# StarRocks/starrocks

Measured on NVIDIA B200. Metric: rows/sec for SSB Q4.1 hash-join+agg, higher is better.
Workload: dtype int32 keys / int64 sums

## Files before the change

### include/sr_gpu_ops.h

```cpp
#ifndef SR_GPU_OPS_H
#define SR_GPU_OPS_H

#include <stddef.h>
#include <stdint.h>

#ifdef __cplusplus
extern "C" {
#endif

#define SR_ABI_VERSION 1

typedef enum sr_status {
    SR_OK = 0,
    SR_ERR_INVALID_ARGUMENT = -1,
    SR_ERR_NOT_SUPPORTED = -2,
    SR_ERR_OUT_OF_MEMORY = -3,
    SR_ERR_CUDA = -4,
    SR_ERR_STATE = -5,
    SR_ERR_NO_DEVICE = -6
} sr_status;

typedef enum sr_type {
    SR_TYPE_BOOLEAN = 1,
    SR_TYPE_TINYINT = 2,
// ... 299 lines not shown
typedef struct sr_frag_join {
    sr_join* join;
    int32_t probe_key_slot;
    int32_t num_payload;
    int32_t payload_build_slots[SR_MAX_FRAG_PAYLOAD];
} sr_frag_join;

typedef struct sr_fragment_desc {
    sr_scan_desc scan;
    int32_t num_joins;
    int32_t mode_hint;
    sr_frag_join joins[SR_MAX_FRAG_JOINS];
    sr_agg_desc agg;
} sr_fragment_desc;

typedef struct sr_fragment sr_fragment;

sr_fragment* sr_fragment_create(sr_ctx* ctx, const sr_fragment_desc* desc);
void sr_fragment_destroy(sr_fragment* frag);
int32_t sr_fragment_push(sr_fragment* frag, const sr_chunk_view* fact);
sr_agg* sr_fragment_agg(sr_fragment* frag);
typedef struct sr_fragment_plan {
    int32_t num_joins;
    int32_t order[SR_MAX_FRAG_JOINS];
    int32_t bitmap_in_smem[SR_MAX_FRAG_JOINS];
    double pass_rate[SR_MAX_FRAG_JOINS];
    int32_t smem_bytes;
    int32_t grid;
    int32_t block;
    int32_t agg_in_smem;
    int32_t mode;
    int32_t num_stream_joins;
    int32_t num_gather_passes;
    int32_t reserved;
    double pred_rate;
} sr_fragment_plan;
int32_t sr_fragment_get_plan(sr_fragment* frag, sr_fragment_plan* plan);
int32_t sr_fragment_last_pass_ms(sr_fragment* frag, float ms[3]);
int32_t sr_fragment_reset(sr_fragment* frag);
int64_t sr_fragment_rows_passed(sr_fragment* frag);

typedef enum sr_hash_fn { SR_HASH_FNV = 0, SR_HASH_CRC32 = 1, SR_HASH_XXH3 = 2 } sr_hash_fn;
typedef enum sr_reduce_op { SR_REDUCE_MULHI = 0 , SR_REDUCE_MODULO = 1  } sr_reduce_op;

#define SR_MAX_PART_KEYS 4

typedef struct sr_part_desc {
    int32_t hash_fn;
    int32_t reduce_op;
    int32_t num_channels;
    int32_t num_part_slots;
    int32_t part_slots[SR_MAX_PART_KEYS];
} sr_part_desc;

typedef struct sr_xchg sr_xchg;

sr_xchg* sr_xchg_create(sr_ctx* ctx, const sr_part_desc* desc);
void sr_xchg_destroy(sr_xchg* x);
int32_t sr_xchg_partition(sr_xchg* x, const sr_chunk_view* in, sr_chunk_out* out, int64_t* channel_offsets_host);
int32_t sr_xchg_hash(sr_xchg* x, const sr_chunk_view* in, uint32_t* hash_values, uint32_t* channel_ids, int32_t mem);

typedef enum sr_page_encoding {
    SR_PAGE_PLAIN = 0,
    SR_PAGE_FOR = 1
} sr_page_encoding;

typedef struct sr_page_view {
// ... 52 lines not shown
```

### starrocks_b200/abi.py

```python
import ctypes as C

import numpy as np

SR_ABI_VERSION = 1

SR_OK = 0
SR_ERR_INVALID_ARGUMENT = -1
SR_ERR_NOT_SUPPORTED = -2
SR_ERR_OUT_OF_MEMORY = -3
SR_ERR_CUDA = -4
SR_ERR_STATE = -5
SR_ERR_NO_DEVICE = -6

TYPE_BOOLEAN, TYPE_TINYINT, TYPE_SMALLINT, TYPE_INT, TYPE_BIGINT, TYPE_LARGEINT = 1, 2, 3, 4, 5, 6
TYPE_FLOAT, TYPE_DOUBLE, TYPE_DATE, TYPE_DATETIME = 7, 8, 9, 10
TYPE_DECIMAL32, TYPE_DECIMAL64, TYPE_DECIMAL128 = 11, 12, 13

TYPE_WIDTH = {
    TYPE_BOOLEAN: 1, TYPE_TINYINT: 1, TYPE_SMALLINT: 2, TYPE_INT: 4, TYPE_BIGINT: 8, TYPE_LARGEINT: 16,
    TYPE_FLOAT: 4, TYPE_DOUBLE: 8, TYPE_DATE: 4, TYPE_DATETIME: 8, TYPE_DECIMAL32: 4, TYPE_DECIMAL64: 8,
    TYPE_DECIMAL128: 16,
}
TYPE_NUMPY = {
    TYPE_BOOLEAN: np.uint8, TYPE_TINYINT: np.int8, TYPE_SMALLINT: np.int16, TYPE_INT: np.int32,
# ... 101 lines not shown
    _fields_ = [("method", C.c_int32), ("has_duplicates", C.c_int32), ("build_rows", C.c_int64),
                ("bucket_size", C.c_int64), ("min_value", C.c_int64), ("max_value", C.c_int64)]


class sr_agg_fn(C.Structure):
    _fields_ = [("kind", C.c_int32), ("input_type", C.c_int32), ("out_slot", C.c_int32), ("reserved", C.c_int32),
                ("input", sr_expr)]


class sr_agg_desc(C.Structure):
    _fields_ = [("num_group_keys", C.c_int32), ("group_slots", C.c_int32 * SR_MAX_GROUP_KEYS),
                ("group_types", C.c_int32 * SR_MAX_GROUP_KEYS), ("has_ranges", C.c_int32),
                ("group_nullable", C.c_int32 * SR_MAX_GROUP_KEYS),
                ("group_min", C.c_int64 * SR_MAX_GROUP_KEYS), ("group_max", C.c_int64 * SR_MAX_GROUP_KEYS),
                ("num_fns", C.c_int32), ("reserved", C.c_int32), ("fns", sr_agg_fn * SR_MAX_AGG_FNS),
                ("expected_groups", C.c_int64)]


class sr_frag_join(C.Structure):
    _fields_ = [("join", C.c_void_p), ("probe_key_slot", C.c_int32), ("num_payload", C.c_int32),
                ("payload_build_slots", C.c_int32 * SR_MAX_FRAG_PAYLOAD)]


class sr_fragment_desc(C.Structure):
    _fields_ = [("scan", sr_scan_desc), ("num_joins", C.c_int32), ("mode_hint", C.c_int32),
                ("joins", sr_frag_join * SR_MAX_FRAG_JOINS), ("agg", sr_agg_desc)]


class sr_fragment_plan(C.Structure):
    _fields_ = [("num_joins", C.c_int32), ("order", C.c_int32 * SR_MAX_FRAG_JOINS),
                ("bitmap_in_smem", C.c_int32 * SR_MAX_FRAG_JOINS), ("pass_rate", C.c_double * SR_MAX_FRAG_JOINS),
                ("smem_bytes", C.c_int32), ("grid", C.c_int32), ("block", C.c_int32), ("agg_in_smem", C.c_int32),
                ("mode", C.c_int32), ("num_stream_joins", C.c_int32), ("num_gather_passes", C.c_int32),
                ("reserved", C.c_int32), ("pred_rate", C.c_double)]


class sr_part_desc(C.Structure):
    _fields_ = [("hash_fn", C.c_int32), ("reduce_op", C.c_int32), ("num_channels", C.c_int32),
                ("num_part_slots", C.c_int32), ("part_slots", C.c_int32 * SR_MAX_PART_KEYS)]


class sr_rf_info(C.Structure):
    _fields_ = [("min_value", C.c_int64), ("max_value", C.c_int64), ("num_inserted", C.c_int64), ("has_null", C.c_int32),
                ("log_num_buckets", C.c_int32), ("key_type", C.c_int32), ("num_in_values", C.c_int32)]


class sr_scan_rf_stats(C.Structure):
    _fields_ = [("rows_tested", C.c_int64), ("rows_passed", C.c_int64), ("batches_skipped", C.c_int64), ("last_selectivity", C.c_double)]


RF_IN_FILTER_ROW_LIMIT = 1024


STATE_REDUCE_SUM, STATE_REDUCE_MIN, STATE_REDUCE_MAX = 0, 1, 2


class sr_agg_state_array(C.Structure):
    _fields_ = [("data", C.c_void_p), ("count", C.c_int64), ("elem_type", C.c_int32), ("reduce", C.c_int32)]


class Chunk:

    def __init__(self, columns, num_rows=None, mem=MEM_HOST):
        self._keep = []
        self.slots = []
        self.types = []
        cols = (sr_col_view * max(1, len(columns)))()
# ... 234 lines not shown
```

### starrocks_b200/csrc/sr_frag.cuh

```cuda
#pragma once

#include "sr_agg.cuh"

#include "sr_frag_kernel.cuh"
#include "sr_frag_pass.cuh"

struct sr_fragment {
    sr_ctx* ctx = nullptr;
    std::vector<sr_pred> preds;
    std::vector<sr_expr> exprs;
    int32_t num_joins = 0;
    sr_frag_join joins[SR_MAX_FRAG_JOINS];
    sr_agg* agg = nullptr;
    bool compiled = false;
    VReg reg;
    std::vector<int32_t> value_src;
    std::vector<const BuildCol*> value_col;
    srd::FragDev host;
    DevBuf dev, counters;
    Staged staged;
    size_t smem_bytes = 0;
    int32_t queue_word_off = 0;
    bool smem_agg = false;
    int grid = 0;
    int order[SR_MAX_FRAG_JOINS];
    double pass_rate[SR_MAX_FRAG_JOINS];
    double pred_rate = 1.0;
    int force_mode = 0;
    bool selective = false;
    bool expand = false;
    srd::PassDev pass;
    std::vector<int> gather_joins;
    DevBuf sel[2], pass_counters;
    double est_rate = 1.0;
    size_t stream_smem = 0;
    int stream_grid = 0;
    int final_grid = 0;
    cudaEvent_t ev[4] = {nullptr, nullptr, nullptr, nullptr};
    bool timed_push = false;
    ~sr_fragment() {
        for (int e = 0; e < 4; e++)
            if (ev[e]) cudaEventDestroy(ev[e]);
    }
};

struct FragTypeCtx {
    sr_fragment* f;
};

static int32_t frag_slot_type(void* user, int32_t slot) {
    sr_fragment* f = ((FragTypeCtx*)user)->f;
    const int k = f->staged.find(slot);
    if (k >= 0) return f->staged.cols[k].type;
    for (int j = 0; j < f->num_joins; j++)
        for (int p = 0; p < f->joins[j].num_payload; p++)
            if (f->joins[j].payload_build_slots[p] == slot) {
                const BuildCol* bc = f->joins[j].join->find_col(slot);
                return bc ? bc->type : 0;
            }
    return 0;
}
static bool frag_slot_nullable(void* user, int32_t slot) {
    sr_fragment* f = ((FragTypeCtx*)user)->f;
    const int k = f->staged.find(slot);
    if (k >= 0) return f->staged.cols[k].nulls != nullptr;
    for (int j = 0; j < f->num_joins; j++)
        for (int p = 0; p < f->joins[j].num_payload; p++)
            if (f->joins[j].payload_build_slots[p] == slot) {
                const BuildCol* bc = f->joins[j].join->find_col(slot);
                return bc && bc->nullable;
// ... 67 lines not shown
        for (size_t k = 0; k < f->agg->reg.slots.size(); k++) {
            remap[k] = merged.add(f->agg->reg.slots[k], f->agg->reg.types[k]);
            if (remap[k] >= SR_MAX_VALUES) return sr_fail(ctx, SR_ERR_NOT_SUPPORTED, "too many distinct columns");
        }
        srd::AggDev& ah = f->agg->host;
        for (int k = 0; k < ah.num_keys; k++) ah.key_value_id[k] = remap[ah.key_value_id[k]];
        for (int q = 0; q < ah.num_fns; q++)
            for (int k = 0; k < ah.fns[q].input.num_nodes; k++)
                if (ah.fns[q].input.nodes[k].op == srd::C_LOAD_I || ah.fns[q].input.nodes[k].op == srd::C_LOAD_D)
                    ah.fns[q].input.nodes[k].arg = remap[ah.fns[q].input.nodes[k].arg];
        f->agg->reg = merged;
        f->reg = merged;
        SR_TRY(agg_upload(f->agg));
    }
    f->value_src.assign(f->reg.slots.size(), -1);
    f->value_col.assign(f->reg.slots.size(), nullptr);
    for (size_t k = 0; k < f->reg.slots.size(); k++) {
        if (f->staged.find(f->reg.slots[k]) >= 0) continue;
        bool found = false;
        for (int j = 0; j < f->num_joins && !found; j++)
            for (int p = 0; p < f->joins[j].num_payload && !found; p++)
                if (f->joins[j].payload_build_slots[p] == f->reg.slots[k]) {
                    f->value_src[k] = j;
                    f->value_col[k] = f->joins[j].join->find_col(f->reg.slots[k]);
                    h.joins[j].need_head = 1;
                    found = true;
                }
        if (!found) return sr_fail(ctx, SR_ERR_INVALID_ARGUMENT, "slot %d is neither a fact column nor a join payload", f->reg.slots[k]);
    }
    SR_TRY(f->counters.reserve(ctx, 256));
    SR_CUDA(ctx, cudaMemsetAsync(f->counters.p, 0, 256, ctx->stream));
    h.rows_passed = f->counters.as<unsigned long long>();
    return SR_OK;
}

static int32_t frag_plan(sr_fragment* f, const VTab& vt, int64_t n) {
    sr_ctx* ctx = f->ctx;
    srd::FragDev& h = f->host;
    SR_TRY(f->dev.reserve(ctx, sizeof(srd::FragDev)));
    SR_CUDA(ctx, cudaMemcpyAsync(f->dev.p, &h, sizeof(h), cudaMemcpyHostToDevice, ctx->stream));
    const int64_t sample = std::min<int64_t>(n, 1 << 16);
    unsigned long long counts[24] = {0};
    static_assert(SR_MAX_FRAG_JOINS + 1 <= 16, "sample counter layout");
    counts[SR_MAX_FRAG_JOINS] = (unsigned long long)sample;
    for (int p = 0; p < 8; p++) counts[16 + p] = (unsigned long long)sample;
    if (sample > 0 && (f->num_joins > 0 || h.num_preds > 0 || h.num_exprs > 0)) {
        unsigned long long* dcounts = f->counters.as<unsigned long long>() + 8;
        SR_CUDA(ctx, cudaMemsetAsync(dcounts, 0, sizeof(counts), ctx->stream));
        srd::k_frag_sample<<<grid_for(sample, 256), 256, 0, ctx->stream>>>((const srd::FragDev*)f->dev.p, vt, sample, dcounts);
        SR_LAUNCH_CHECK(ctx);
        SR_CUDA(ctx, cudaMemcpyAsync(counts, dcounts, sizeof(counts), cudaMemcpyDeviceToHost, ctx->stream));
        SR_CUDA(ctx, cudaStreamSynchronize(ctx->stream));
    }
    for (int j = 0; j < f->num_joins; j++) f->pass_rate[j] = sample > 0 ? (double)counts[j] / (double)sample : 1.0;
    f->pred_rate = sample > 0 ? (double)counts[SR_MAX_FRAG_JOINS] / (double)sample : 1.0;
    std::vector<int> ord(f->num_joins);
    for (int j = 0; j < f->num_joins; j++) ord[j] = j;
    std::stable_sort(ord.begin(), ord.end(), [&](int a, int b) {
        const double pa = f->pass_rate[a], pb = f->pass_rate[b];
        if (std::abs(pa - pb) > 0.15 * std::max(pa, pb)) return pa < pb;
        return h.joins[a].bitmap_words < h.joins[b].bitmap_words;
    });
    srd::FragJoinDev reordered[SR_MAX_FRAG_JOINS];
    std::vector<int> inv(f->num_joins);
    for (int q = 0; q < f->num_joins; q++) {
        reordered[q] = h.joins[ord[q]];
// ... 98 lines not shown
            srd::FragJoinDev& fj = h.joins[q];
            fj.smem_off = -1;
            if (q < ns && fj.use_bitmap && sw + (size_t)fj.bitmap_words + 1 <= sbudget) {
                fj.smem_off = (int32_t)sw;
                sw += ((size_t)fj.bitmap_words + 1 + 3) & ~(size_t)3;
            }
        }
        f->stream_smem = sw * 4;
        f->smem_agg = f->agg->smem_bytes > 0;
        f->smem_bytes = f->agg->smem_bytes;
        f->queue_word_off = 0;
        SR_CUDA(ctx, cudaMemcpyAsync(f->dev.p, &h, sizeof(h), cudaMemcpyHostToDevice, ctx->stream));
        SR_CUDA(ctx, cudaStreamSynchronize(ctx->stream));
        int per_sm = 0;
        SR_CUDA(ctx, cudaFuncSetAttribute(srd::k_frag_stream<false>, cudaFuncAttributeMaxDynamicSharedMemorySize, (int)std::max<size_t>(f->stream_smem, 16)));
        SR_CUDA(ctx, cudaFuncSetAttribute(srd::k_frag_stream<true>, cudaFuncAttributeMaxDynamicSharedMemorySize, (int)std::max<size_t>(f->stream_smem, 16)));
        SR_CUDA(ctx, cudaFuncSetAttribute(srd::k_frag_stream_tests<false>, cudaFuncAttributeMaxDynamicSharedMemorySize, (int)std::max<size_t>(f->stream_smem, 16)));
        SR_CUDA(ctx, cudaFuncSetAttribute(srd::k_frag_stream_tests<true>, cudaFuncAttributeMaxDynamicSharedMemorySize, (int)std::max<size_t>(f->stream_smem, 16)));
        SR_CUDA(ctx, cudaOccupancyMaxActiveBlocksPerMultiprocessor(&per_sm, srd::k_frag_stream<false>, srd::STREAM_BLOCK, f->stream_smem));
        if (per_sm < 1) return sr_fail(ctx, SR_ERR_CUDA, "streaming pass does not fit on an SM (smem %zu)", f->stream_smem);
        f->stream_grid = per_sm * ctx->num_sms;
        int gj = 0, ga = 0;
        SR_CUDA(ctx, cudaOccupancyMaxActiveBlocksPerMultiprocessor(&gj, srd::k_frag_gather_join, srd::GATHER_BLOCK, 0));
        if (f->expand)
            SR_CUDA(ctx, cudaOccupancyMaxActiveBlocksPerMultiprocessor(&ga, srd::k_frag_gather_agg_expand, srd::GATHER_BLOCK, 0));
        else if (f->agg->host.num_keys == 0)
            SR_CUDA(ctx, cudaOccupancyMaxActiveBlocksPerMultiprocessor(&ga, srd::k_frag_gather_agg<false, true>, srd::GATHER_BLOCK, 0));
        else if (f->smem_agg)
            SR_CUDA(ctx, cudaOccupancyMaxActiveBlocksPerMultiprocessor(&ga, srd::k_frag_gather_agg<true>, srd::GATHER_BLOCK, f->agg->smem_bytes));
        else
            SR_CUDA(ctx, cudaOccupancyMaxActiveBlocksPerMultiprocessor(&ga, srd::k_frag_gather_agg<false>, srd::GATHER_BLOCK, 0));
        f->grid = std::max(gj, 1) * ctx->num_sms;
        f->final_grid = std::max(ga, 1) * ctx->num_sms;
        SR_TRY(f->pass_counters.reserve(ctx, 16 * sizeof(uint64_t)));
        f->compiled = true;
        return SR_OK;
    }
    size_t words = 0;
    f->smem_agg = f->agg->smem_bytes > 0;
    if (f->smem_agg) words += (f->agg->smem_bytes + 15) / 16 * 4;
    const size_t budget_words = (96 * 1024) / 4;
    const size_t queue_words = (size_t)srd::FRAG_WARPS * srd::FRAG_WARP_QWORDS;
    for (int q = 0; q < f->num_joins; q++) {
        srd::FragJoinDev& fj = h.joins[q];
        fj.smem_off = -1;
        if (fj.use_bitmap && words + (size_t)fj.bitmap_words + queue_words <= budget_words) {
            fj.smem_off = (int32_t)words;
            words += (size_t)fj.bitmap_words;
            words = (words + 3) & ~(size_t)3;
        }
    }
    f->queue_word_off = (int32_t)words;
    words += queue_words;
    f->smem_bytes = words * 4;
    SR_CUDA(ctx, cudaMemcpyAsync(f->dev.p, &h, sizeof(h), cudaMemcpyHostToDevice, ctx->stream));
    SR_CUDA(ctx, cudaStreamSynchronize(ctx->stream));
    int per_sm = 0;
    SR_CUDA(ctx, cudaFuncSetAttribute(srd::k_fragment<true>, cudaFuncAttributeMaxDynamicSharedMemorySize, (int)f->smem_bytes));
    SR_CUDA(ctx, cudaFuncSetAttribute(srd::k_fragment<false>, cudaFuncAttributeMaxDynamicSharedMemorySize, (int)f->smem_bytes));
    if (f->smem_agg)
        SR_CUDA(ctx, cudaOccupancyMaxActiveBlocksPerMultiprocessor(&per_sm, srd::k_fragment<true>, srd::FRAG_BLOCK, f->smem_bytes));
    else
        SR_CUDA(ctx, cudaOccupancyMaxActiveBlocksPerMultiprocessor(&per_sm, srd::k_fragment<false>, srd::FRAG_BLOCK, f->smem_bytes));
    if (per_sm < 1) return sr_fail(ctx, SR_ERR_CUDA, "fragment kernel does not fit on an SM (smem %zu)", f->smem_bytes);
    f->grid = per_sm * ctx->num_sms;
    f->compiled = true;
    return SR_OK;
}

static int32_t frag_push(sr_fragment* f, const sr_chunk_view* fact) {
    sr_ctx* ctx = f->ctx;
    if (f->agg->finished) return sr_fail(ctx, SR_ERR_STATE, "fragment push after sink_finish");
    if (fact->num_rows >= 0xFFFFFFF0ll) return sr_fail(ctx, SR_ERR_NOT_SUPPORTED, "fragment batch of more than 2^32 rows; push smaller morsels");
    SR_TRY(f->staged.stage(ctx, fact, nullptr, true));
    const int64_t n = fact->num_rows;
    bool first = !f->compiled;
    if (first) SR_TRY(frag_compile(f));
    VTab vt;
    SR_TRY(frag_bind_vtab(f, &vt));
    if (first) {
        SR_TRY(frag_plan(f, vt, n));
        SR_TRY(frag_bind_vtab(f, &vt));
    }
    if (n == 0) return SR_OK;
    SR_TRY(agg_check_nullability(f->agg, vt));
// ... 21 lines not shown
        if (!carry) pass.carry_join = pass.carry_value_id = -1;
        unsigned long long* cnt = f->pass_counters.as<unsigned long long>();
        SR_CUDA(ctx, cudaMemsetAsync(cnt, 0, 16 * sizeof(uint64_t), ctx->stream));
        const int sgrid = (int)std::min<int64_t>(f->stream_grid, (n + srd::STREAM_TILE - 1) / srd::STREAM_TILE);
        if (!f->ev[0])
            for (int e = 0; e < 4; e++) SR_CUDA(ctx, cudaEventCreate(&f->ev[e]));
        SR_CUDA(ctx, cudaEventRecord(f->ev[0], ctx->stream));
        bool tests = pass.num_tests > 0;
        for (int t = 0; t < pass.num_tests && tests; t++) {
            const VDesc& d = vt.v[pass.tests[t].value_id];
            if (d.nulls != nullptr || (t < pass.num_vec && (((uintptr_t)d.data) & 15) != 0)) tests = false;
        }
        static const bool use_tma = getenv("SR_FRAG_STREAM_TMA") != nullptr;
        if (tests && use_tma && !pass.host_input) {
            const uint32_t bitmap_bytes = (uint32_t)((f->stream_smem + 127) / 128 * 128);
            const size_t sm = bitmap_bytes + srd::STREAM_TMA_SMEM;
            SR_CUDA(ctx, cudaFuncSetAttribute(srd::k_frag_stream_tests_tma<false>, cudaFuncAttributeMaxDynamicSharedMemorySize, (int)sm));
            int per_sm = 1;
            SR_CUDA(ctx, cudaOccupancyMaxActiveBlocksPerMultiprocessor(&per_sm, srd::k_frag_stream_tests_tma<false>, srd::STREAM_BLOCK, sm));
            const int tgrid = (int)std::min<int64_t>((int64_t)std::max(per_sm, 1) * ctx->num_sms, (n + srd::STREAM_TILE - 1) / srd::STREAM_TILE);
            srd::k_frag_stream_tests_tma<false><<<tgrid, srd::STREAM_BLOCK, sm, ctx->stream>>>(fdev, pass, vt, n, bitmap_bytes, f->sel[0].as<srd::SelEntry>(), cnt);
        } else if (tests) {
            if (carry)
                srd::k_frag_stream_tests<true><<<sgrid, srd::STREAM_BLOCK, f->stream_smem, ctx->stream>>>(fdev, pass, vt, n, f->sel[0].as<srd::SelEntry>(), cnt);
            else
                srd::k_frag_stream_tests<false><<<sgrid, srd::STREAM_BLOCK, f->stream_smem, ctx->stream>>>(fdev, pass, vt, n, f->sel[0].as<srd::SelEntry>(), cnt);
        } else if (carry) {
            srd::k_frag_stream<true><<<sgrid, srd::STREAM_BLOCK, f->stream_smem, ctx->stream>>>(fdev, pass, vt, n, f->sel[0].as<srd::SelEntry>(), cnt);
        } else {
            srd::k_frag_stream<false><<<sgrid, srd::STREAM_BLOCK, f->stream_smem, ctx->stream>>>(fdev, pass, vt, n, f->sel[0].as<srd::SelEntry>(), cnt);
        }
        SR_LAUNCH_CHECK(ctx);
        SR_CUDA(ctx, cudaEventRecord(f->ev[1], ctx->stream));
        int cur = 0, k = 0;
        for (int q : f->gather_joins) {
            srd::k_frag_gather_join<<<f->grid, srd::GATHER_BLOCK, 0, ctx->stream>>>(fdev, q, vt, f->sel[cur].as<srd::SelEntry>(), cnt + k,
                                                                                  f->sel[cur ^ 1].as<srd::SelEntry>(), cnt + k + 1);
            SR_LAUNCH_CHECK(ctx);
            cur ^= 1;
            k++;
        }
        SR_CUDA(ctx, cudaEventRecord(f->ev[2], ctx->stream));
        if (hash) SR_TRY(f->sel[cur ^ 1].reserve(ctx, sizeof(srd::SelEntry) * ((size_t)n + slack)));
        srd::SelEntry* fail_list = hash ? f->sel[cur ^ 1].as<srd::SelEntry>() : nullptr;
        unsigned long long* fail_count = cnt + 8;
        if (f->expand)
            srd::k_frag_gather_agg_expand<<<f->final_grid, srd::GATHER_BLOCK, 0, ctx->stream>>>(fdev, (const srd::AggDev*)a->dev.p, pass, vt,
                                                                                       f->sel[cur].as<srd::SelEntry>(), cnt + k, fail_list, fail_count);
        else if (ah.num_keys == 0)
            srd::k_frag_gather_agg<false, true><<<f->final_grid, srd::GATHER_BLOCK, 0, ctx->stream>>>(fdev, (const srd::AggDev*)a->dev.p, pass, vt,
                                                                                              f->sel[cur].as<srd::SelEntry>(), cnt + k, nullptr, nullptr);
        else if (f->smem_agg)
            srd::k_frag_gather_agg<true><<<f->final_grid, srd::GATHER_BLOCK, a->smem_bytes, ctx->stream>>>(fdev, (const srd::AggDev*)a->dev.p, pass, vt,
                                                                                                   f->sel[cur].as<srd::SelEntry>(), cnt + k, nullptr, nullptr);
        else
            srd::k_frag_gather_agg<false><<<f->final_grid, srd::GATHER_BLOCK, 0, ctx->stream>>>(fdev, (const srd::AggDev*)a->dev.p, pass, vt,
                                                                                        f->sel[cur].as<srd::SelEntry>(), cnt + k, fail_list, fail_count);
        SR_LAUNCH_CHECK(ctx);
        SR_CUDA(ctx, cudaEventRecord(f->ev[3], ctx->stream));
        f->timed_push = true;
        if (hash) {
            int fc = 8;
            while (true) {
                uint64_t ng;
                int32_t ovf, bad;
                SR_CUDA(ctx, cudaMemcpyAsync(ctx->pinned + 16, cnt + fc, 8, cudaMemcpyDeviceToHost, ctx->stream));
                SR_TRY(agg_read_counters(a, &ng, &ovf, &bad));
                a->ngroups_host = (int64_t)ng;
                const uint64_t failed = ctx->pinned[16];
                if (failed == 0) break;
                SR_CUDA(ctx, cudaMemsetAsync((uint8_t*)a->counters.p + 8, 0, 8, ctx->stream));
                uint64_t cap = a->host.cap * 2;
                while ((uint64_t)a->ngroups_host + failed > cap / 2) cap *= 2;
                if (cap > (1ull << 33)) return sr_fail(ctx, SR_ERR_OUT_OF_MEMORY, "aggregate table would exceed 2^33 slots; push smaller batches");
                SR_TRY(agg_grow(a, cap));
                cur ^= 1;
                const int nfc = fc == 8 ? 9 : 8;
                SR_CUDA(ctx, cudaMemsetAsync(cnt + nfc, 0, 8, ctx->stream));
                if (f->expand)
// ... 31 lines not shown
```

### starrocks_b200/csrc/sr_frag_pass.cuh

```cuda
#pragma once

#include "sr_frag_kernel.cuh"

namespace srd {

struct StreamTest {
    int32_t kind;
    int32_t value_id;
    int32_t join;
    uint32_t lo, span;
};
#define SR_MAX_STREAM_TESTS 6

struct PassDev {
    int32_t num_tests;
    int32_t num_vec;
    StreamTest tests[SR_MAX_STREAM_TESTS];
    int32_t num_stream_joins;
    int32_t final_first_join;
    int8_t final_vals[8];
    int8_t final_slot[SR_MAX_VALUES];
    int8_t host_input;
    int8_t carry_join;
    int8_t carry_value_id;
// ... 692 lines not shown
                if (test && head == 0) ok = false;
            } else if (test) {
                if (!join_hit_global(fj, key)) ok = false;
            }
        }
        if (!ok) continue;
        if (single) {
            single_acc_row(ad, sacc, ld);
        } else if (hash_table) {
            HKey key;
            agg_pack_key(ad, ld, key);
            bool inserted;
            const long long slot = agg_find_slot_key(ad, key, inserted, known_groups);
            agg_count_new_groups(ad, inserted, known_groups);
            if (slot < 0) {
                if (fail_list) fail_list[atomicAdd(fail_count, 1ull)] = entry;
                continue;
            }
            agg_apply_row<SMEM_AGG>(ad, acc, slot, ld);
        } else {
            const long long slot = agg_find_slot(ad, ld);
            if (slot >= 0) agg_apply_row<SMEM_AGG>(ad, acc, slot, ld);
        }
        passed++;
    }
    __syncwarp();
    if (single) single_acc_flush(ad, sacc);
    if (SMEM_AGG) {
        __syncthreads();
        acc_smem_flush(ad, acc);
    }
    passed = warp_sum(passed);
    if (lane_id() == 0 && passed) atomicAdd(fd.rows_passed, passed);
}

__global__ void __launch_bounds__(GATHER_BLOCK) k_frag_gather_agg_expand(const FragDev* __restrict__ fdp, const AggDev* __restrict__ adp, const __grid_constant__ PassDev pd,
                                                                          const __grid_constant__ VTab vt, const SelEntry* __restrict__ sel_in,
                                                                          const unsigned long long* __restrict__ n_in_ptr, SelEntry* __restrict__ fail_list,
                                                                          unsigned long long* __restrict__ fail_count) {
    __shared__ FragJoinDev s_joins[SR_MAX_FRAG_JOINS];
    const FragDev& fd = *fdp;
    const AggDev& ad = *adp;
    const int S = fd.num_joins;
    const bool single = ad.num_keys == 0;
    const bool hash_table = !ad.dense && ad.num_keys > 0;
    unsigned long long known_groups = hash_table && fail_list ? *(volatile unsigned long long*)ad.ngroups : 0ull;
    for (int i = threadIdx.x; i < (int)(sizeof(FragJoinDev) / 4) * S; i += blockDim.x) ((uint32_t*)s_joins)[i] = ((const uint32_t*)fd.joins)[i];
    AccPtrs acc;
    acc_ptrs_global(ad, acc);
    __syncthreads();
    const unsigned long long n_in = *n_in_ptr;
    unsigned long long passed = 0;
    SingleAcc sacc;
    if (single) single_acc_init(ad, sacc);
    unsigned long long w_begin, w_end;
    warp_sel_range(n_in, w_begin, w_end);
    for (unsigned long long i = w_begin + lane_id(); i < w_end; i += 32) {
        const SelEntry entry = sel_in[i];
        const uint32_t row = sel_row(entry);
        if (row == SEL_INVALID) continue;
        FragLoader ld{vt, (int64_t)row, {0, 0, 0, 0, 0, 0}, pd.carry_join >= 0 ? (int32_t)pd.carry_value_id : -1, sel_carry(entry)};
        uint32_t head[SR_MAX_FRAG_JOINS];
        bool ok = true;
#pragma unroll 1
        for (int j = 0; j < S && ok; j++) {
            const FragJoinDev& fj = s_joins[j];
// ... 69 lines not shown
```

### starrocks_b200/csrc/sr_gpu.cu

```cuda
#include "sr_frag.cuh"
#include "sr_serde.cuh"
#include "sr_page.cuh"

namespace srd {

struct PartCols {
    DCol c[SR_MAX_PART_KEYS];
    int32_t n;
    int32_t hash_fn;
    int32_t reduce;
    int32_t num_channels;
};

__device__ __forceinline__ uint32_t part_hash_row(const PartCols& pc, int64_t row) {
    uint32_t h = pc.hash_fn == SR_HASH_FNV ? 0x811C9DC5u : pc.hash_fn == SR_HASH_XXH3 ? 0x9E3779B1u : 0u;
    for (int k = 0; k < pc.n; k++) {
        const DCol& c = pc.c[k];
        if (c.nulls && c.nulls[row]) {
            if (pc.hash_fn == SR_HASH_CRC32)
                h = zlib_crc32_bytes(0, 0, 4, h);
            else
                h = h ^ (0x9e3779b9u + (h << 6) + (h >> 2));
            continue;
        }
// ... 1271 lines not shown
    delete frag->agg;
    delete frag;
}

int32_t sr_fragment_push(sr_fragment* frag, const sr_chunk_view* fact) {
    if (!frag || !fact) return SR_ERR_INVALID_ARGUMENT;
    SR_BIND(frag->ctx);
    return frag_push(frag, fact);
}

sr_agg* sr_fragment_agg(sr_fragment* frag) {
    return frag ? frag->agg : nullptr;
}

int32_t sr_fragment_get_plan(sr_fragment* frag, sr_fragment_plan* plan) {
    if (!frag || !plan) return SR_ERR_INVALID_ARGUMENT;
    SR_LOCK(frag->ctx);
    if (!frag->compiled) return sr_fail(frag->ctx, SR_ERR_STATE, "the fragment plans on its first push");
    memset(plan, 0, sizeof(*plan));
    plan->num_joins = frag->num_joins;
    for (int q = 0; q < frag->num_joins; q++) {
        plan->order[q] = frag->order[q];
        plan->bitmap_in_smem[q] = frag->host.joins[q].smem_off >= 0 ? 1 : 0;
        plan->pass_rate[q] = frag->pass_rate[q];
    }
    plan->smem_bytes = (int32_t)frag->smem_bytes;
    plan->grid = frag->grid;
    plan->block = srd::FRAG_BLOCK;
    plan->agg_in_smem = frag->smem_agg ? 1 : 0;
    plan->mode = frag->selective ? 2 : 1;
    plan->num_stream_joins = frag->selective ? frag->pass.num_stream_joins : 0;
    plan->num_gather_passes = frag->selective ? (int32_t)frag->gather_joins.size() : 0;
    plan->pred_rate = frag->pred_rate;
    if (frag->selective) {
        plan->smem_bytes = (int32_t)frag->stream_smem;
        plan->grid = frag->stream_grid;
        plan->block = srd::STREAM_BLOCK;
    }
    return SR_OK;
}

int32_t sr_fragment_last_pass_ms(sr_fragment* frag, float ms[3]) {
    if (!frag || !ms) return SR_ERR_INVALID_ARGUMENT;
    sr_ctx* ctx = frag->ctx;
    SR_BIND(ctx);
    if (!frag->timed_push) return sr_fail(ctx, SR_ERR_STATE, "no timed push (selection-vector mode only)");
    SR_CUDA(ctx, cudaEventSynchronize(frag->ev[3]));
    for (int k = 0; k < 3; k++) SR_CUDA(ctx, cudaEventElapsedTime(&ms[k], frag->ev[k], frag->ev[k + 1]));
    return SR_OK;
}

int32_t sr_fragment_reset(sr_fragment* frag) {
    if (!frag) return SR_ERR_INVALID_ARGUMENT;
    sr_ctx* ctx = frag->ctx;
    SR_BIND(ctx);
    SR_TRY(agg_reset_impl(frag->agg));
    if (frag->compiled) SR_CUDA(ctx, cudaMemsetAsync(frag->counters.p, 0, 8, ctx->stream));
    return SR_OK;
}

int64_t sr_fragment_rows_passed(sr_fragment* frag) {
    if (!frag) return SR_ERR_INVALID_ARGUMENT;
    sr_ctx* ctx = frag->ctx;
    SR_BIND(ctx);
    if (!frag->compiled) return 0;
    SR_CUDA(ctx, cudaMemcpyAsync(ctx->pinned + 16, frag->counters.p, 8, cudaMemcpyDeviceToHost, ctx->stream));
// ... 273 lines not shown
```

### starrocks_b200/gpu.py

```python
import ctypes as C
import os
import subprocess

import numpy as np

from . import abi

_HERE = os.path.dirname(os.path.abspath(__file__))
LIB_PATH = os.environ.get("SR_GPU_LIB") or os.path.join(_HERE, "libsr_gpu.so")
_LIB = None

NVCC_FLAGS = ["-gencode", "arch=compute_100a,code=sm_100a", "-O3", "-lineinfo", "-std=c++17", "-shared",
              "-Xcompiler", "-fPIC", "-cudart", "static"]


def _source_files():
    csrc = os.path.join(_HERE, "csrc")
    return sorted(os.path.join(csrc, f) for f in os.listdir(csrc)) + [os.path.join(_HERE, "..", "include", "sr_gpu_ops.h")]


def _source_hash():
    import hashlib
    h = hashlib.sha256()
    for f in _source_files():
# ... 442 lines not shown
    def num_groups(self):
        return self.ctx.check(lib().sr_agg_num_groups(self.h))

    def pull(self, max_rows=1 << 62, mem=abi.MEM_HOST):
        out = abi.sr_chunk_out()
        self.ctx.check(lib().sr_agg_pull(self.h, max_rows, mem, C.byref(out)))
        return out

    def result(self):
        self.finish()
        out = self.pull()
        return chunk_out_to_host(self.ctx, out)


def two_phase_descs(desc):
    p1, p2 = abi.sr_agg_desc(), abi.sr_agg_desc()
    rc = lib().sr_agg_two_phase_descs(C.byref(desc), C.byref(p1), C.byref(p2))
    if rc != 0:
        raise GpuError(rc, "sr_agg_two_phase_descs: the aggregate cannot be split into two phases (128-bit states or too many functions)")
    return p1, p2


def chunk_out_as_view(out):
    class _View:
        pass
    v = _View()
    v.view = abi.sr_chunk_view(C.cast(out.cols, C.POINTER(abi.sr_col_view)), out.num_cols, out.mem, out.num_rows)
    v.num_rows = out.num_rows
    v._keep = out
    v.ref = lambda: C.byref(v.view)
    return v


class Fragment:
    def __init__(self, ctx, scan_desc, joins, agg_desc, mode=0):
        self.ctx = ctx
        self._keep = (scan_desc, joins, agg_desc)
        d = abi.sr_fragment_desc()
        d.scan = scan_desc.desc
        d.num_joins = len(joins)
        d.mode_hint = mode
        for k, (j, slot, payload) in enumerate(joins):
            d.joins[k].join = j.h
            d.joins[k].probe_key_slot = slot
            d.joins[k].num_payload = len(payload)
            for q, s in enumerate(payload):
                d.joins[k].payload_build_slots[q] = s
        d.agg = agg_desc
        self.desc = d
        self.h = lib().sr_fragment_create(ctx.h, C.byref(d))
        if not self.h:
            ctx.check(lib().sr_last_error_code(ctx.h) or -1)
        self.agg = Agg(ctx, agg_desc, handle=lib().sr_fragment_agg(self.h))

    def close(self):
        if self.h:
            lib().sr_fragment_destroy(self.h)
            self.h = None

    def push(self, chunk):
        self.ctx.check(lib().sr_fragment_push(self.h, chunk.ref()))

    def reset(self):
        self.ctx.check(lib().sr_fragment_reset(self.h))

    def last_pass_ms(self):
        ms = (C.c_float * 3)()
        rc = lib().sr_fragment_last_pass_ms(self.h, ms)
        if rc == abi.SR_ERR_STATE:
            return None
        self.ctx.check(rc)
        return [float(x) for x in ms]

    def plan(self):
        p = abi.sr_fragment_plan()
        self.ctx.check(lib().sr_fragment_get_plan(self.h, C.byref(p)))
        nj = p.num_joins
        return {"order": list(p.order[:nj]), "bitmap_in_smem": list(p.bitmap_in_smem[:nj]),
                "pass_rate": [round(x, 4) for x in p.pass_rate[:nj]], "smem_bytes": p.smem_bytes, "grid": p.grid,
                "block": p.block, "agg_in_smem": bool(p.agg_in_smem),
                "mode": {1: "fused-cascade", 2: "selection-vector-passes"}.get(p.mode, p.mode),
                "num_stream_joins": p.num_stream_joins, "num_gather_passes": p.num_gather_passes,
                "pred_rate": round(p.pred_rate, 4)}

    @property
    def rows_passed(self):
        return self.ctx.check(lib().sr_fragment_rows_passed(self.h))


def chunk_serialize(ctx, chunk, row_begin=0, row_end=None):
    row_end = chunk.num_rows if row_end is None else row_end
    n = ctx.check(lib().sr_chunk_serialized_size(chunk.ref(), row_begin, row_end))
    buf = np.zeros(n, dtype=np.uint8)
    meta = abi.sr_chunk_pb_meta()
    ctx.check(lib().sr_chunk_serialize(ctx.h, chunk.ref(), row_begin, row_end, buf.ctypes.data, n, abi.MEM_HOST, C.byref(meta)))
    return buf, meta


class PageDecoder:

    def __init__(self, ctx):
        self.ctx = ctx
        self.h = lib().sr_page_decoder_create(ctx.h)

    def close(self):
        if self.h:
            lib().sr_page_decoder_destroy(self.h)
            self.h = None

    def decode(self, encoding, typ, pages, out_ptr, out_capacity, mem=abi.MEM_HOST):
        views = (abi.sr_page_view * max(1, len(pages)))()
        keep = []
        for k, pg in enumerate(pages):
            if isinstance(pg, tuple):
                views[k].data, views[k].size = pg
            else:
# ... 52 lines not shown
```

Measured before the change: 279.7 billion.

## Add specialized plain final gather-agg kernel for dense int32 selective fragments

Adds a specialized final-stage kernel for the selection-vector path. It applies when the remaining joins are direct-mapped int32 bitmap or first-index joins, the group keys are dense, and the aggregates are only COUNT or SUM_I64. The kernel batches R rows per lane, issues predicated loads for columns, join heads and payloads, and accumulates into a shared-memory dense table that is merged with global atomics at the end. It replaces the generic interpreted gather-agg to cut per-row dispatch and register overhead, at the cost of a large new code path with its own eligibility checks that must stay consistent with the generic path.

```diff
diff --git a/include/sr_gpu_ops.h b/include/sr_gpu_ops.h
--- a/include/sr_gpu_ops.h
+++ b/include/sr_gpu_ops.h
@@ -355,7 +355,7 @@
     int32_t mode;
     int32_t num_stream_joins;
     int32_t num_gather_passes;
-    int32_t reserved;
+    int32_t final_kind;
     double pred_rate;
 } sr_fragment_plan;
 int32_t sr_fragment_get_plan(sr_fragment* frag, sr_fragment_plan* plan);
diff --git a/starrocks_b200/abi.py b/starrocks_b200/abi.py
--- a/starrocks_b200/abi.py
+++ b/starrocks_b200/abi.py
@@ -157,7 +157,7 @@
                 ("bitmap_in_smem", C.c_int32 * SR_MAX_FRAG_JOINS), ("pass_rate", C.c_double * SR_MAX_FRAG_JOINS),
                 ("smem_bytes", C.c_int32), ("grid", C.c_int32), ("block", C.c_int32), ("agg_in_smem", C.c_int32),
                 ("mode", C.c_int32), ("num_stream_joins", C.c_int32), ("num_gather_passes", C.c_int32),
-                ("reserved", C.c_int32), ("pred_rate", C.c_double)]
+                ("final_kind", C.c_int32), ("pred_rate", C.c_double)]
 
 
 class sr_part_desc(C.Structure):
diff --git a/starrocks_b200/csrc/sr_frag.cuh b/starrocks_b200/csrc/sr_frag.cuh
--- a/starrocks_b200/csrc/sr_frag.cuh
+++ b/starrocks_b200/csrc/sr_frag.cuh
@@ -36,6 +36,8 @@
     size_t stream_smem = 0;
     int stream_grid = 0;
     int final_grid = 0;
+    int final_kind = 0;
+    srd::PlainFinalDev plain;
     cudaEvent_t ev[4] = {nullptr, nullptr, nullptr, nullptr};
     bool timed_push = false;
     ~sr_fragment() {
@@ -169,6 +171,107 @@
     SR_CUDA(ctx, cudaMemsetAsync(f->counters.p, 0, 256, ctx->stream));
     h.rows_passed = f->counters.as<unsigned long long>();
     return SR_OK;
+}
+
+static bool vt_plain32_value(const VTab& vt, int id) {
+    const VDesc& d = vt.v[id];
+    return d.nulls == nullptr && (d.type == SR_TYPE_INT || d.type == SR_TYPE_DATE || d.type == SR_TYPE_DECIMAL32);
+}
+
+static bool frag_plan_plain(sr_fragment* f, const VTab& vt, int ff) {
+    const srd::FragDev& h = f->host;
+    const srd::AggDev& ah = f->agg->host;
+    srd::PlainFinalDev& p = f->plain;
+    memset(&p, 0, sizeof(p));
+    p.carry_slot = -1;
+    if (f->expand || !f->smem_agg || !ah.dense || ah.num_keys == 0 || ah.num_fns > SR_MAX_AGG_FNS) return false;
+    int cols[PLAIN_MAX_COLS], joins[PLAIN_MAX_JOINS];
+    int nc = 0, nj = 0, np = 0;
+    for (int q = 0; q < f->num_joins; q++) {
+        const srd::FragJoinDev& fj = h.joins[q];
+        if (!fj.need_head && q < ff) continue;
+        if (nj == PLAIN_MAX_JOINS || !fj.use_bitmap || !fj.idx32 || fj.expand || !vt_plain32_value(vt, fj.key_value_id)) return false;
+        for (int c = 0; c < nc; c++)
+            if (cols[c] == fj.key_value_id) return false;
+        joins[nj++] = q;
+        cols[nc++] = fj.key_value_id;
+    }
+    auto source = [&](int id) -> int {
+        if (id < 0 || id >= (int)f->value_src.size() || !vt_plain32_value(vt, id)) return -1;
+        if (f->value_src[id] < 0) {
+            for (int c = 0; c < nc; c++)
+                if (cols[c] == id) return c;
+            if (nc == PLAIN_MAX_COLS) return -1;
+            cols[nc] = id;
+            return nc++;
+        }
+        for (int k = 0; k < np; k++)
+            if (p.payload_value_id[k] == id) return PLAIN_SRC_PAYLOAD + k;
+        int pj = -1;
+        for (int k = 0; k < nj; k++)
+            if (joins[k] == f->value_src[id]) pj = k;
+        if (np == PLAIN_MAX_PAYLOADS || pj < 0) return -1;
+        p.payload_value_id[np] = (int8_t)id;
+        p.payload_join[np] = (int8_t)pj;
+        return PLAIN_SRC_PAYLOAD + np++;
+    };
+    for (int k = 0; k < ah.num_keys; k++) {
+        if (ah.key_nullable[k]) return false;
+        const int s = source(ah.key_value_id[k]);
+        if (s < 0) return false;
+        p.key_src[k] = (int8_t)s;
+        p.dense_min[k] = ah.dense_min[k];
+        p.dense_extent[k] = ah.dense_extent[k];
+        p.dense_stride[k] = ah.dense_stride[k];
+    }
+    uint32_t off = 1;
+    for (int q = 0; q < ah.num_fns; q++) {
+        const srd::AggFnDev& fn = ah.fns[q];
+        p.fn_src[q] = -1;
+        if (fn.mode == srd::M_COUNT_STAR) {
+            p.fn_kind[q] = 0;
+            continue;
+        }
+        if ((fn.mode != srd::M_COUNT && fn.mode != srd::M_SUM_I64) || fn.track_n || fn.n_value_id >= 0 || fn.input.num_nodes != 1 ||
+            fn.input.nodes[0].op != srd::C_LOAD_I)
+            return false;
+        const int s = source(fn.input.nodes[0].arg);
+        if (s < 0) return false;
+        p.fn_kind[q] = fn.mode == srd::M_COUNT ? 1 : 2;
+        p.fn_src[q] = (int8_t)s;
+        p.fn_off[q] = off++;
+    }
+    if ((size_t)off * ah.cap * 8 != f->agg->smem_bytes) return false;
+    for (int k = 0; k < nj; k++) {
+        const srd::FragJoinDev& fj = h.joins[joins[k]];
+        srd::PlainJoin& pj = p.join[k];
+        pj.first = fj.need_head ? fj.j.first : nullptr;
+        pj.bitmap = fj.j.bitmap;
+        pj.umin = (uint32_t)(int32_t)fj.j.min_value;
+        pj.span = (uint32_t)(fj.j.max_value - fj.j.min_value);
+        pj.test = joins[k] >= ff ? 1 : 0;
+    }
+    for (int c = 0; c < nc; c++) p.col_value_id[c] = (int8_t)cols[c];
+    p.num_cols = nc;
+    p.num_joins = nj;
+    p.num_payloads = np;
+    p.num_keys = ah.num_keys;
+    p.num_fns = ah.num_fns;
+    p.cap = (uint32_t)ah.cap;
+    p.rows_passed = h.rows_passed;
+    p.bad_key_flag = ah.flags + 1;
+    return true;
+}
+
+static bool frag_plain_bind(const sr_fragment* f, const VTab& vt, const srd::PassDev& pass, srd::PlainFinalDev& p) {
+    p = f->plain;
+    for (int c = 0; c < p.num_cols; c++) {
+        if (!vt_plain32_value(vt, p.col_value_id[c])) return false;
+        p.col[c] = (const int32_t*)vt.v[p.col_value_id[c]].data;
+        if (pass.carry_join >= 0 && p.col_value_id[c] == pass.carry_value_id) p.carry_slot = c;
+    }
+    for (int k = 0; k < p.num_payloads; k++) p.payload[k] = (const int32_t*)vt.v[p.payload_value_id[k]].data;
+    return true;
 }
 
 static int32_t frag_plan(sr_fragment* f, const VTab& vt, int64_t n) {
@@ -333,6 +436,13 @@
             SR_CUDA(ctx, cudaOccupancyMaxActiveBlocksPerMultiprocessor(&ga, srd::k_frag_gather_agg<false>, srd::GATHER_BLOCK, 0));
         f->grid = std::max(gj, 1) * ctx->num_sms;
         f->final_grid = std::max(ga, 1) * ctx->num_sms;
+        f->final_kind = 1;
+        if (frag_plan_plain(f, vt, ff)) {
+            f->final_kind = 2;
+            int gp = 0;
+            SR_CUDA(ctx, cudaOccupancyMaxActiveBlocksPerMultiprocessor(&gp, srd::k_frag_final_plain<SR_FINAL_PLAIN_ROWS>, srd::GATHER_BLOCK, f->agg->smem_bytes));
+            f->final_grid = std::max(gp, 1) * ctx->num_sms;
+        }
         SR_TRY(f->pass_counters.reserve(ctx, 16 * sizeof(uint64_t)));
         f->compiled = true;
         return SR_OK;
@@ -352,6 +462,7 @@
         }
     }
     f->queue_word_off = (int32_t)words;
+    f->final_kind = 0;
     words += queue_words;
     f->smem_bytes = words * 4;
     SR_CUDA(ctx, cudaMemcpyAsync(f->dev.p, &h, sizeof(h), cudaMemcpyHostToDevice, ctx->stream));
@@ -439,6 +550,8 @@
         }
         SR_LAUNCH_CHECK(ctx);
         SR_CUDA(ctx, cudaEventRecord(f->ev[1], ctx->stream));
+        srd::PlainFinalDev plain;
+        const bool use_plain = f->final_kind == 2 && f->smem_agg && frag_plain_bind(f, vt, pass, plain);
         int cur = 0, k = 0;
         for (int q : f->gather_joins) {
             srd::k_frag_gather_join<<<f->grid, srd::GATHER_BLOCK, 0, ctx->stream>>>(fdev, q, vt, f->sel[cur].as<srd::SelEntry>(), cnt + k,
@@ -451,7 +564,10 @@
         if (hash) SR_TRY(f->sel[cur ^ 1].reserve(ctx, sizeof(srd::SelEntry) * ((size_t)n + slack)));
         srd::SelEntry* fail_list = hash ? f->sel[cur ^ 1].as<srd::SelEntry>() : nullptr;
         unsigned long long* fail_count = cnt + 8;
-        if (f->expand)
+        if (use_plain)
+            srd::k_frag_final_plain<SR_FINAL_PLAIN_ROWS><<<f->final_grid, srd::GATHER_BLOCK, a->smem_bytes, ctx->stream>>>(
+                    plain, (const srd::AggDev*)a->dev.p, f->sel[cur].as<srd::SelEntry>(), cnt + k);
+        else if (f->expand)
             srd::k_frag_gather_agg_expand<<<f->final_grid, srd::GATHER_BLOCK, 0, ctx->stream>>>(fdev, (const srd::AggDev*)a->dev.p, pass, vt,
                                                                                        f->sel[cur].as<srd::SelEntry>(), cnt + k, fail_list, fail_count);
         else if (ah.num_keys == 0)
diff --git a/starrocks_b200/csrc/sr_frag_pass.cuh b/starrocks_b200/csrc/sr_frag_pass.cuh
--- a/starrocks_b200/csrc/sr_frag_pass.cuh
+++ b/starrocks_b200/csrc/sr_frag_pass.cuh
@@ -748,6 +748,177 @@
     }
     passed = warp_sum(passed);
     if (lane_id() == 0 && passed) atomicAdd(fd.rows_passed, passed);
+}
+
+#define PLAIN_MAX_COLS 6
+#define PLAIN_MAX_JOINS 4
+#define PLAIN_MAX_PAYLOADS 4
+#define PLAIN_SRC_PAYLOAD 8
+
+struct PlainJoin {
+    const uint32_t* first;
+    const uint32_t* bitmap;
+    uint32_t umin, span;
+    int32_t test;
+    int32_t pad;
+};
+
+struct PlainFinalDev {
+    const int32_t* col[PLAIN_MAX_COLS];
+    const int32_t* payload[PLAIN_MAX_PAYLOADS];
+    PlainJoin join[PLAIN_MAX_JOINS];
+    long long dense_min[SR_MAX_GROUP_KEYS];
+    long long dense_extent[SR_MAX_GROUP_KEYS];
+    long long dense_stride[SR_MAX_GROUP_KEYS];
+    uint32_t fn_off[SR_MAX_AGG_FNS];
+    int32_t num_cols, num_joins, num_payloads, num_keys, num_fns;
+    int32_t carry_slot;
+    uint32_t cap;
+    int8_t col_value_id[PLAIN_MAX_COLS];
+    int8_t payload_value_id[PLAIN_MAX_PAYLOADS];
+    int8_t payload_join[PLAIN_MAX_PAYLOADS];
+    int8_t key_src[SR_MAX_GROUP_KEYS];
+    int8_t fn_src[SR_MAX_AGG_FNS];
+    int8_t fn_kind[SR_MAX_AGG_FNS];
+    int8_t pad[4];
+    unsigned long long* rows_passed;
+    int32_t* bad_key_flag;
+};
+
+#ifndef SR_FINAL_PLAIN_ROWS
+#define SR_FINAL_PLAIN_ROWS 2
+#endif
+#ifndef SR_FINAL_PLAIN_MIN_BLOCKS
+#define SR_FINAL_PLAIN_MIN_BLOCKS 4
+#endif
+
+__device__ __forceinline__ int32_t select_eq(int32_t s, int32_t c, int32_t a, int32_t x) {
+    int32_t r;
+    asm("{ .reg .pred q; setp.eq.s32 q, %1, %2; selp.b32 %0, %3, %4, q; }" : "=r"(r) : "r"(s), "r"(c), "r"(a), "r"(x));
+    return r;
+}
+
+__device__ __forceinline__ int32_t plain_src(int32_t s, const int32_t (&v)[PLAIN_MAX_COLS], const int32_t (&pv)[PLAIN_MAX_PAYLOADS]) {
+    int32_t x = 0;
+#pragma unroll
+    for (int c = 0; c < PLAIN_MAX_COLS; c++) x = select_eq(s, c, v[c], x);
+#pragma unroll
+    for (int q = 0; q < PLAIN_MAX_PAYLOADS; q++) x = select_eq(s, PLAIN_SRC_PAYLOAD + q, pv[q], x);
+    return x;
+}
+
+template <int R>
+__global__ void __launch_bounds__(GATHER_BLOCK, SR_FINAL_PLAIN_MIN_BLOCKS) k_frag_final_plain(const __grid_constant__ PlainFinalDev p, const AggDev* __restrict__ adp,
+                                                                                            const SelEntry* __restrict__ sel_in,
+                                                                                            const unsigned long long* __restrict__ n_in_ptr) {
+    extern __shared__ __align__(16) uint32_t smem[];
+    long long* const sacc = (long long*)smem;
+    uint32_t words = p.cap;
+#pragma unroll
+    for (int f = 0; f < SR_MAX_AGG_FNS; f++)
+        if (f < p.num_fns && p.fn_kind[f] != 0) words += p.cap;
+    for (uint32_t i = threadIdx.x; i < words; i += blockDim.x) sacc[i] = 0;
+    __syncthreads();
+    const unsigned long long n_in = *n_in_ptr;
+    unsigned long long w_begin, w_end;
+    warp_sel_range(n_in, w_begin, w_end);
+    uint32_t passed = 0;
+    bool bad_key = false;
+    for (unsigned long long i0 = w_begin; i0 < w_end; i0 += 32 * R) {
+        uint32_t row[R];
+        int32_t carry[R];
+        bool live[R];
+#pragma unroll
+        for (int r = 0; r < R; r++) {
+            const unsigned long long i = i0 + r * 32 + lane_id();
+            const SelEntry e = i < w_end ? sel_in[i] : (SelEntry)SEL_INVALID;
+            row[r] = sel_row(e);
+            carry[r] = sel_carry(e);
+            live[r] = row[r] != SEL_INVALID;
+        }
+        int32_t v[R][PLAIN_MAX_COLS];
+#pragma unroll
+        for (int c = 0; c < PLAIN_MAX_COLS; c++)
+#pragma unroll
+            for (int r = 0; r < R; r++) {
+                v[r][c] = 0;
+                if (c < p.num_cols) {
+                    const int32_t x = ldg_stream_s32_pred(p.col[c] + row[r], live[r] && c != p.carry_slot);
+                    v[r][c] = select_eq(c, p.carry_slot, carry[r], x);
+                }
+            }
+        uint32_t b[R][PLAIN_MAX_JOINS];
+#pragma unroll
+        for (int q = 0; q < PLAIN_MAX_JOINS; q++)
+#pragma unroll
+            for (int r = 0; r < R; r++) {
+                b[r][q] = 0;
+                if (q < p.num_joins) {
+                    const uint32_t idx = (uint32_t)v[r][q] - p.join[q].umin;
+                    const bool in = live[r] && idx <= p.join[q].span;
+                    b[r][q] = p.join[q].first ? ldg_u32_pred(p.join[q].first + idx, in) : ldg_u32_pred(p.join[q].bitmap + (idx >> 5), in);
+                }
+            }
+#pragma unroll
+        for (int q = 0; q < PLAIN_MAX_JOINS; q++)
+#pragma unroll
+            for (int r = 0; r < R; r++)
+                if (q < p.num_joins) {
+                    if (!p.join[q].first) b[r][q] = (b[r][q] >> (((uint32_t)v[r][q] - p.join[q].umin) & 31)) & 1u;
+                    if (p.join[q].test && b[r][q] == 0) live[r] = false;
+                }
+        int32_t pv[R][PLAIN_MAX_PAYLOADS];
+#pragma unroll
+        for (int k = 0; k < PLAIN_MAX_PAYLOADS; k++)
+#pragma unroll
+            for (int r = 0; r < R; r++) {
+                pv[r][k] = 0;
+                if (k < p.num_payloads) {
+                    uint32_t bi = 0;
+#pragma unroll
+                    for (int q = 0; q < PLAIN_MAX_JOINS; q++) bi = (uint32_t)select_eq(p.payload_join[k], q, (int32_t)b[r][q], (int32_t)bi);
+                    pv[r][k] = (int32_t)ldg_u32_pred((const uint32_t*)p.payload[k] + bi, live[r]);
+                }
+            }
+#pragma unroll
+        for (int r = 0; r < R; r++) {
+            if (!live[r]) continue;
+            passed++;
+            uint32_t slot = 0;
+            bool bad = false;
+#pragma unroll
+            for (int k = 0; k < SR_MAX_GROUP_KEYS; k++)
+                if (k < p.num_keys) {
+                    const long long idx = (long long)plain_src(p.key_src[k], v[r], pv[r]) - p.dense_min[k];
+                    bad |= idx < 0 || idx >= p.dense_extent[k];
+                    slot += (uint32_t)idx * (uint32_t)p.dense_stride[k];
+                }
+            if (bad) {
+                bad_key = true;
+                continue;
+            }
+            smem_add_u64(sacc + slot, 1ull);
+#pragma unroll
+            for (int f = 0; f < SR_MAX_AGG_FNS; f++)
+                if (f < p.num_fns && p.fn_kind[f] != 0) {
+                    const unsigned long long add = p.fn_kind[f] == 1 ? 1ull : (unsigned long long)(long long)plain_src(p.fn_src[f], v[r], pv[r]);
+                    smem_add_u64(sacc + p.fn_off[f] * p.cap + slot, add);
+                }
+        }
+    }
+    if (bad_key) *p.bad_key_flag = 1;
+    __syncthreads();
+    const AggDev& ad = *adp;
+    for (uint32_t i = threadIdx.x; i < p.cap; i += blockDim.x) {
+        const long long c = sacc[i];
+        if (c == 0) continue;
+        atomicAdd((unsigned long long*)ad.cnt_star + i, (unsigned long long)c);
+#pragma unroll
+        for (int f = 0; f < SR_MAX_AGG_FNS; f++)
+            if (f < p.num_fns && p.fn_kind[f] != 0) acc_merge(ad.fns[f].mode, ad.fns[f].acc0, nullptr, i, sacc[p.fn_off[f] * p.cap + i], 0);
+    }
+    const unsigned long long total = warp_sum((unsigned long long)passed);
+    if (lane_id() == 0 && total) atomicAdd(p.rows_passed, total);
 }
 
 __global__ void __launch_bounds__(GATHER_BLOCK) k_frag_gather_agg_expand(const FragDev* __restrict__ fdp, const AggDev* __restrict__ adp, const __grid_constant__ PassDev pd,
diff --git a/starrocks_b200/csrc/sr_gpu.cu b/starrocks_b200/csrc/sr_gpu.cu
--- a/starrocks_b200/csrc/sr_gpu.cu
+++ b/starrocks_b200/csrc/sr_gpu.cu
@@ -1327,6 +1327,7 @@
     plan->num_stream_joins = frag->selective ? frag->pass.num_stream_joins : 0;
     plan->num_gather_passes = frag->selective ? (int32_t)frag->gather_joins.size() : 0;
     plan->pred_rate = frag->pred_rate;
+    plan->final_kind = frag->final_kind;
     if (frag->selective) {
         plan->smem_bytes = (int32_t)frag->stream_smem;
         plan->grid = frag->stream_grid;
diff --git a/starrocks_b200/gpu.py b/starrocks_b200/gpu.py
--- a/starrocks_b200/gpu.py
+++ b/starrocks_b200/gpu.py
@@ -498,6 +498,9 @@
     return v
 
 
+FINAL_KINDS = {0: "k_fragment", 1: "k_frag_gather_agg", 2: "k_frag_final_plain"}
+
+
 class Fragment:
     def __init__(self, ctx, scan_desc, joins, agg_desc, mode=0):
         self.ctx = ctx
@@ -547,7 +550,7 @@
                 "block": p.block, "agg_in_smem": bool(p.agg_in_smem),
                 "mode": {1: "fused-cascade", 2: "selection-vector-passes"}.get(p.mode, p.mode),
                 "num_stream_joins": p.num_stream_joins, "num_gather_passes": p.num_gather_passes,
-                "pred_rate": round(p.pred_rate, 4)}
+                "final": FINAL_KINDS.get(p.final_kind, p.final_kind), "pred_rate": round(p.pred_rate, 4)}
 
     @property
     def rows_passed(self):
```

Measured after the change: 291.9 billion (median of 6 runs). 4.4% higher.
